# shivams15/navierstokessolver

Hardware: AMD Instinct MI355X
Metric: cell-updates/sec (MLUPS) + Poisson iters/sec, 4096^2 grid at 1/2/4/8 GPUs (higher is better)
Workload: dtype f64

## Files before the change

navierstokessolver_amd/csrc/ns_fps.hip:

```cpp
#include <hip/hip_ext.h>
#include <hip/hip_runtime.h>

#include <algorithm>

#include "ns_internal.h"

namespace nsg {

namespace {

struct cplx {
    double x, y;
};
__device__ inline cplx cadd(cplx a, cplx b) { return {a.x + b.x, a.y + b.y}; }
__device__ inline cplx csub(cplx a, cplx b) { return {a.x - b.x, a.y - b.y}; }
__device__ inline cplx cmul(cplx a, cplx b) { return {fma(a.x, b.x, -a.y * b.y), fma(a.x, b.y, a.y * b.x)}; }

__device__ inline double2 ld2(const double* p) { return *reinterpret_cast<const double2*>(p); }
__device__ inline void st2(double* p, double x, double y) { *reinterpret_cast<double2*>(p) = double2{x, y}; }

__device__ constexpr double C16[8] = {1.0, 0.92387953251128675613, 0.70710678118654752440, 0.38268343236508977173,
                                      0.0, -0.38268343236508977173, -0.70710678118654752440, -0.92387953251128675613};
__device__ constexpr double S16[8] = {0.0, 0.38268343236508977173, 0.70710678118654752440, 0.92387953251128675613,
                                      1.0, 0.92387953251128675613, 0.70710678118654752440, 0.38268343236508977173};
// ... 1351 lines not shown
        BR[w][0] = BR[w][1] = 1.0;
        if (c < a.nch) {
            double2 e = le[w];
            const double2 pp = lp[w];
            double2 bl = lb[w];
            if (a.m0e && k0 == 0) {
                const double sft = a.ny * *a.m0s;
                e.x -= sft * a.m0e[c];
                bl.x -= sft * a.m0b[c];
            }
            const double2 be = lbe[w], br = lbr[w];
            if (!a.mid_local) st2(a.ya + (size_t)c * a.ld + k0, Y[0], Y[1]);
            BX[w][0] = fma(be.x, Y[0], bl.x);
            BX[w][1] = fma(be.y, Y[1], bl.y);
            BR[w][0] = br.x;
            BR[w][1] = br.y;
            if (!a.mid_local) st2(a.cb + (size_t)c * a.ld + k0, BX[w][0], BX[w][1]);
            Y[0] = fma(pp.x, Y[0], e.x);
            Y[1] = fma(pp.y, Y[1], e.y);
        }
    }
    double GX[2] = {0.0, 0.0}, GR[2] = {1.0, 1.0};
#pragma unroll
    for (int w = FPS_G - 1; w >= 0; w--) {
        GX[0] = fma(BR[w][0], GX[0], BX[w][0]);
        GX[1] = fma(BR[w][1], GX[1], BX[w][1]);
        GR[0] = BR[w][0] * GR[0];
        GR[1] = BR[w][1] * GR[1];
    }
    st2(a.gb + (size_t)grp * a.ld + k0, GX[0], GX[1]);
    st2(a.gb + (size_t)(a.ngrp + grp) * a.ld + k0, GR[0], GR[1]);
}

template <bool GHOST>
__global__ void __launch_bounds__(64 * FPS_G) k_fps_t2b(FpsArgs a, double* __restrict__ f) {
    const int lane = threadIdx.x, w = __builtin_amdgcn_readfirstlane(threadIdx.y);
    const int k0 = 2 * (blockIdx.x * 64 + lane);
    const int grp = blockIdx.y, c = grp * FPS_G + w;
    const int li0 = c * FPS_M;
    const int rows = k0 < a.ny ? min(FPS_M, a.nxl - li0) : 0;
    ChunkRows cr;
    cr.load_wave(a, li0);
    if (rows <= 0) return;
    const double s0 = mode0_shift(a, k0);
    double2 yv[FPS_M];
#pragma unroll
    for (int t = 0; t < FPS_M; t++)
        yv[t] = ldf0(a, f, min(li0 + t, a.nxl - 1), k0, s0);
    const double2 yin = ld2(a.ya + (size_t)c * a.ld + k0);
    const double2 x0 = ld2(a.gx + (size_t)grp * a.ld + k0);
    double X[2] = {x0.x, x0.y};
    for (int q = FPS_G - 1; q > w; q--) {
        const int cq = grp * FPS_G + q;
        if (cq >= a.nch) continue;
        const double2 bx = ld2(a.cb + (size_t)cq * a.ld + k0), br = ld2(a.bt + (size_t)(a.nch + cq) * a.ld + k0);
        X[0] = fma(br.x, X[0], bx.x);
        X[1] = fma(br.y, X[1], bx.y);
    }
    if (GHOST && c == a.nch - 1 && a.i0 + a.nxl < a.nx) st2(f + (size_t)a.nxl * a.ld + k0, X[0], X[1]);
    const double mu[2] = {a.mu[k0], a.mu[k0 + 1]};
    const double2 r0 = ld2(a.rp0 + (size_t)c * a.ld + k0);
    double r[2] = {r0.x, r0.y}, y[2] = {yin.x, yin.y};
    double2 rv[FPS_M];
    const int pb = fps_prow_block(a);
    const bool fast = pb < a.nx;
    const double2 pinf = fast ? ld2(a.pinf + k0) : double2{0.0, 0.0};
// ... 529 lines not shown
    }
    if (a.cnt <= 0) return np;
    int n = -1;
    switch (lg) {
    case 4: n = div_pair<4>(k, a, st); break;
    case 5: n = div_pair<5>(k, a, st); break;
    case 6: n = div_pair<6>(k, a, st); break;
    case 7: n = div_pair<7>(k, a, st); break;
    case 8: n = div_pair<8>(k, a, st); break;
    case 9: n = div_pair<9>(k, a, st); break;
    case 10: n = div_pair<10>(k, a, st); break;
    case 11: n = div_pair<11>(k, a, st); break;
    case 12: n = div_pair<12>(k, a, st); break;
    case 13: n = div_pair<13>(k, a, st); break;
    default: return -1;
    }
    return n < 0 ? -1 : np;
}

bool fps_fuse_ok(const Knobs& k, int ny, int outE) { return ny == (1 << 14) ? fps_div_real(k, 14, outE) : fps_log2(ny) >= 0; }

void launch_fps_t1(const FpsArgs& a, const double* f, hipStream_t st) {
    hipLaunchKernelGGL(k_fps_t1, dim3((a.ny + 127) / 128, a.ngrp), dim3(64, FPS_G), 0, st, a, f);
}
void launch_fps_t2(const FpsArgs& a, double* f, hipStream_t st) {
    hipLaunchKernelGGL(k_fps_t2, dim3((a.ny + 127) / 128, a.ngrp), dim3(64, FPS_G), 0, st, a, f);
}
void launch_fps_t1b(const FpsArgs& a, const double* f, hipStream_t st) {
    hipLaunchKernelGGL(k_fps_t1b, dim3((a.ny + 127) / 128, a.ngrp), dim3(64, FPS_G), 0, st, a, f);
}
void launch_fps_mid(const FpsArgs& a, const double* f, hipStream_t st) {
    hipLaunchKernelGGL(k_fps_mid, dim3((a.ny + 127) / 128, a.ngrp), dim3(64), 0, st, a, f);
}
namespace {
__global__ void k_fps_oe_s0(const double* __restrict__ f, int row, int ld, int last, double* __restrict__ out) {
    if (threadIdx.x == 0) out[0] = last ? 2.0 * f[(size_t)row * ld] : 0.0;
}
}
void launch_fps_oe_s0(const double* f, int row, int ld, int last, double* out, hipStream_t st) {
    hipLaunchKernelGGL(k_fps_oe_s0, dim3(1), dim3(64), 0, st, f, row, ld, last, out);
}
void launch_fps_t2b(const FpsArgs& a, double* f, hipStream_t st) {
    if (a.ghost) hipLaunchKernelGGL(k_fps_t2b<true>, dim3((a.ny + 127) / 128, a.ngrp), dim3(64, FPS_G), 0, st, a, f);
    else hipLaunchKernelGGL(k_fps_t2b<false>, dim3((a.ny + 127) / 128, a.ngrp), dim3(64, FPS_G), 0, st, a, f);
}
void launch_fps_t3(const FpsArgs& a, double* f, hipStream_t st) {
    hipLaunchKernelGGL(k_fps_t3, dim3((a.ny + 127) / 128, a.ngrp), dim3(64, FPS_G), 0, st, a, f);
}
namespace {

__global__ __launch_bounds__(256) void k_cap_gemv(CapArgs a, const double* __restrict__ z) {
    extern __shared__ double gl[];
    const int M = a.m + a.border;
    for (int f = threadIdx.x; f < M; f += 256) gl[f] = f < a.m ? z[a.fi[f]] - z[a.fj[f]] : 0.0;
    __syncthreads();
    const int row = blockIdx.x * 4 + (threadIdx.x >> 6), lane = threadIdx.x & 63;
    if (row >= M) return;
    const double* cr = a.cinv + (size_t)row * M;
    double acc = 0.0;
    for (int k = lane; k < M; k += 64) acc = fma(cr[k], gl[k], acc);
    for (int off = 32; off > 0; off >>= 1) acc += __shfl_xor(acc, off, 64);
    if (lane == 0) a.y[row] = acc;
}

__global__ __launch_bounds__(256) void k_cap_scatter(CapArgs a, double* __restrict__ q, int mode) {
    const int c = blockIdx.x * 256 + threadIdx.x;
// ... 125 lines not shown
```

navierstokessolver_amd/csrc/ns_internal.h:

```cpp
#pragma once
#include <hip/hip_runtime.h>
#include <cstdint>
#include <vector>

#include "ns_knobs.h"

namespace nsg {

constexpr int HALO = 7;

constexpr int FC_IN = 1 << 20;
constexpr int FC_DEEP = 1 << 21;
constexpr int FC_BAND = 1 << 22;
constexpr int FC_INT = 31;
constexpr int MAX_EDGES = 31;
__host__ __device__ inline int fc_edge(int code, int k) { return (code >> (5 * k)) & 31; }
struct EdgeDev {
    int neu;
    int enx, eny;
    double c0, c1;
};

struct Geo {
    const int32_t* fc = nullptr;
    const EdgeDev* et = nullptr;
    int nx, ny;
    int i0, nxl;
    int ld;
    int neu[4];
    double c0[4], c1[4];
    int enx[4], eny[4];
    int sr0 = 0, sr1 = 1 << 30;
    int dsx = 0;
    const int* ecell = nullptr;
    int necell = 0;
};

struct Coef {
// ... 39 lines not shown
int launch_helm_sweep3(const Knobs& kn, const Geo& g, const Coef& c, double alpha, double omega, const double* u, const double* v,
                       double* uo, double* vo, const double* ru, const double* rv, hipStream_t st, int which,
                       double* part = nullptr);
int launch_helm_sweep2(const Knobs& kn, const Geo& g, const Coef& c, double alpha, double omega, const double* u, const double* v,
                       double* uo, double* vo, const double* ru, const double* rv, double* part, hipStream_t st,
                       int which = 3);

int launch_pois_rbsor_tiled(const Geo& g, const Coef& c, double omega, const double* phi, double* out,
                            const double* rp, const double* shift, double* part, hipStream_t st);
int launch_pois_jacobi_tiled(const Geo& g, const Coef& c, double omega, const double* in, double* out,
                             const double* rp, const double* shift, double* part, hipStream_t st);
void set_strip_rows(int L);
void set_compute_cus(int n);
int device_cus();
void lds_attr_once(const void* kern, int bytes);
void time_next_launch(hipEvent_t a, hipEvent_t b);
bool time_next_launch_pending();
bool take_launch_timing(hipEvent_t& a, hipEvent_t& b);
void set_strip_phase(int phase);
int launch_pois_residual(const Geo& g, const Coef& c, const double* phi, const double* rp,
                         const double* shift, double* part, hipStream_t st);
int launch_correct(const Knobs& kn, const Geo& g, const Coef& c, double dt, const double* us, const double* vs, double* u, double* v,
                   const double* phi, double* part, hipStream_t st);
bool correct_streams(const Knobs& kn, const Geo& g);
int launch_correct_guess(const Knobs& kn, const Geo& g, const Coef& c, double dt, const double* us, const double* vs, double* u,
                         double* v, const double* phi, double* part, const double* h1, const double* h2,
                         const double* h3, const double* gc, double* gout, hipStream_t st);
void launch_reduce_sum(const double* p, int n, int nv, double* out, hipStream_t st);
void launch_reduce_sum_segs(const double* p, int n, int nseg, double* out, hipStream_t st);
void launch_reduce_sum_min(const double* ps, int ns, int nvs, double* outs, const double* pm, int nm, int nvm,
                           double* outm, hipStream_t st);
void launch_reduce_min(const double* p, int n, int nv, double* out, hipStream_t st);
void launch_reduce_sum_mean(const double* p, int n, double* sums, double ncells, double* out, hipStream_t st);
void launch_finish_mean(const double* sums, double ncells, double* shift_and_bn2, hipStream_t st);
void launch_bus_reduce(const double* gathered, int P, int nv, int nsum, const int* dst, double* out, hipStream_t st);
int launch_sums(const Geo& g, const double* f, double* part, hipStream_t st);
void launch_axpby(const Geo& g, double a, const double* x, double b, const double* y, double* out, hipStream_t st,
                  double c = 0.0, const double* z = nullptr, double d = 0.0, const double* w = nullptr,
                  double e = 0.0, const double* v = nullptr);
int launch_area_sum(const Geo& g, const Coef& c, const double* b, double* part, hipStream_t st);
void launch_area_fix(const Geo& g, const Coef& c, double* b, const double* sab, const double* shift, double area,
                     double inv_area, double n, double* kshift, hipStream_t st);
void launch_fill_random(const Geo& g, double* phi, double* rp, uint64_t seed, hipStream_t st);


__host__ __device__ inline bool mg_can_coarsen(int nx, int ny) {
    return nx % 2 == 0 && ny % 2 == 0 && nx >= 4 && ny >= 4 && nx * ny > 16;
}

int launch_restrict(const Geo& gf, const Coef& cf, const double* phi, const double* b, const double* shift,
                    const Geo& gc, const Coef& cc, double* bc, double* pc, double* part, hipStream_t st);
void launch_prolong(const Geo& gf, double* phi, const Geo& gc, const double* ec, hipStream_t st);

int launch_pois_rbsor2_restrict(const Knobs& kn, const Geo& g, const Coef& c, double omega, const double* phi, double* out,
                                const double* rp, const double* shift, const Geo& gc, double* bc, double* pc,
                                double* part, hipStream_t st, bool zin = false);

int launch_pois_rbsor2_restrict_guess(const Knobs& kn, const Geo& g, const Coef& c, double omega, const double* phi, double* out,
                                      const double* rp, const double* shift, const Geo& gc, double* bc, double* pc,
                                      double* part, const double* h1, const double* h2, const double* h3,
                                      const double* gcoef, hipStream_t st);

int launch_pois_rbsor2_prolong(const Knobs& kn, const Geo& g, const Coef& c, double omega, const double* phi, double* out,
                               const double* rp, const double* shift, const Geo& gc, const double* ec,
                               double* part, hipStream_t st);

// ... 78 lines not shown
    double* s0 = nullptr;
    int s0_given = 0;
    const double *ptab = nullptr, *pinf = nullptr;
    int prow = 0, kfast = 1 << 30;
    const int* prowb = nullptr;
    int mid_local = 0;
    int ghost = 0;
};
struct FpsRank {
    const double* gath = nullptr;
    int P = 1, r = 0, stride = 0;
    const double *a1 = nullptr, *ge1 = nullptr;
    double ncells = 0.0;
    double* shift = nullptr;
    const double *bq = nullptr, *x1 = nullptr;
};
int fps_log2(int ny);
bool fps_idct_mask_ok(int ny);
bool fps_fuse_ok(const Knobs& kn, int ny, int outE);
int launch_fps_idct_masked(const Knobs& kn, const double* in, double* out, int nrows, int ny, int ld, const double* tw, const double* wk,
                           hipStream_t st, const int32_t* fcm);
int launch_fps_dct(const Knobs& kn, bool inverse, const double* in, const double* shift, double* out, int nrows, int ny, int ld,
                   const double* tw, const double* wk, hipStream_t st, int oe_pair = -1, const double* tw8 = nullptr);
int fps_log2x(int ny);
bool fps_gen_ok(int ny);
void launch_dense_mats(const double* C, const double* shy, double rsum, int N, double* F, double* G, hipStream_t st);
int launch_fps_div(const Knobs& kn, const Geo& g, const Coef& c, double dt, const double* u, const double* v, double* b, double* out,
                   double* part, int phase, const double* tw, const double* wk, hipStream_t st, int outE = 0);
void launch_fps_t1(const FpsArgs& a, const double* f, hipStream_t st);
void launch_fps_t2(const FpsArgs& a, double* f, hipStream_t st);
void launch_fps_t3(const FpsArgs& a, double* f, hipStream_t st);
void launch_fps_t1b(const FpsArgs& a, const double* f, hipStream_t st);
void launch_fps_mid(const FpsArgs& a, const double* f, hipStream_t st);
void launch_fps_t2b(const FpsArgs& a, double* f, hipStream_t st);
void launch_fps_oe_s0(const double* f, int row, int ld, int last, double* out, hipStream_t st);
void launch_fps_scan(const FpsArgs& a, bool backward, const FpsRank& R, double* rout, hipStream_t st);

struct CapArgs {
    int m = 0, ncell = 0, border = 0;
    const double* e1 = nullptr;
    const int *fi = nullptr, *fj = nullptr, *fk = nullptr, *fm = nullptr, *co = nullptr;
    const int4* cf = nullptr;
    const double* w = nullptr;
    double *cinv = nullptr, *y = nullptr;
};
constexpr size_t CAP_LDS_MAX = 8192;
hipError_t launch_cap_gemv(const CapArgs& a, const double* z, hipStream_t st);
void launch_cap_scatter(const CapArgs& a, double* q, int mode, hipStream_t st);
void launch_cap_axpy(const Geo& g, const CapArgs& a, double* x, const double* z, int set, hipStream_t st);
void launch_cap_fill(const Geo& g, double* q, double val, hipStream_t st);
void launch_cap_rhs(const Geo& g, const double* b, const double* shift, double* r, hipStream_t st);
void launch_cap_src(const CapArgs& a, double* q, int fprev, int f, hipStream_t st);
void launch_cap_col(const CapArgs& a, const double* z, int f, double* cmat, hipStream_t st);
void launch_gj_invert(double* A, int m, double* t, double* u, double* flag, int spd, hipStream_t st);

}
```

navierstokessolver_amd/csrc/ns_kernels.hip:

```cpp
#include "ns_internal.h"
#include <hip/hip_ext.h>

#include <cmath>
#include <cstdio>
#include <cstdlib>
#include <cstring>
#include <map>
#include <set>
#include <mutex>

#include <algorithm>

namespace nsg {

#ifndef LANE_DPP
#define LANE_DPP 1
#endif
__device__ __forceinline__ double lane_up1(double x) {
#if LANE_DPP
    const int lo = __double2loint(x), hi = __double2hiint(x);
    return __hiloint2double(__builtin_amdgcn_update_dpp(hi, hi, 0x138, 0xf, 0xf, false),
                            __builtin_amdgcn_update_dpp(lo, lo, 0x138, 0xf, 0xf, false));
#else
    return __shfl_up(x, 1, 64);
// ... 3804 lines not shown
    double m[4] = {INFINITY, INFINITY, INFINITY, INFINITY};
    for (int k = threadIdx.x; k < n; k += 1024)
#pragma unroll
        for (int v = 0; v < 4; v++)
            if (v < nv) m[v] = fmin(m[v], p[(size_t)k * nv + v]);
#pragma unroll
    for (int v = 0; v < 4; v++)
#pragma unroll
        for (int off = 32; off > 0; off >>= 1) m[v] = fmin(m[v], __shfl_xor(m[v], off, 64));
    const int wv = threadIdx.x >> 6, lane = threadIdx.x & 63;
    if (lane == 0)
#pragma unroll
        for (int v = 0; v < 4; v++) sh[wv][v] = m[v];
    __syncthreads();
    if (threadIdx.x < 4 && (int)threadIdx.x < nv) {
        double r = sh[0][threadIdx.x];
        for (int w = 1; w < 16; w++) r = fmin(r, sh[w][threadIdx.x]);
        out[threadIdx.x] = r;
    }
}
__global__ __launch_bounds__(1024) void k_reduce_min(const double* __restrict__ p, int n, int nv,
                                                     double* __restrict__ out) {
    __shared__ double sh[16][4];
    reduce_min_body(p, n, nv, out, sh);
}
__global__ __launch_bounds__(1024) void k_reduce_sum_min(const double* __restrict__ ps, int ns, int nvs,
                                                         double* __restrict__ outs, const double* __restrict__ pm,
                                                         int nm, int nvm, double* __restrict__ outm) {
    __shared__ double sh[1024];
    if (blockIdx.x == 0) reduce_sum_body(ps, ns, nvs, outs, sh);
    else reduce_min_body(pm, nm, nvm, outm, reinterpret_cast<double (*)[4]>(sh));
}

__global__ __launch_bounds__(1024) void k_reduce_sum_mean(const double* __restrict__ p, int n,
                                                          double* __restrict__ sums, double nc,
                                                          double* __restrict__ out) {
    __shared__ double sh[1024];
    double r[2];
    for (int v = 0; v < 2; v++) {
        double s = 0.0;
        for (int k = threadIdx.x; k < n; k += 1024) s += p[(size_t)k * 2 + v];
        r[v] = tree_sum_1024(s, sh);
        if (threadIdx.x == 0) sums[v] = r[v];
    }
    if (threadIdx.x == 0) {
        const double s = r[0], s2 = r[1];
        out[0] = s / nc;
        out[1] = fmax(s2 - s * s / nc, 0.0);
    }
}
__global__ void k_finish_mean(const double* __restrict__ sums, double n, double* __restrict__ out) {
    const double s = sums[0], s2 = sums[1];
    out[0] = s / n;
    out[1] = fmax(s2 - s * s / n, 0.0);
}

struct BusDst {
    int d[16];
};
__global__ void k_bus_reduce(const double* __restrict__ g, int P, int nv, int nsum, BusDst dst,
                             double* __restrict__ out) {
    const int t = threadIdx.x;
    if (t >= nv) return;
    double a = g[t];
    for (int q = 1; q < P; q++) {
        const double x = g[(size_t)q * nv + t];
// ... 1686 lines not shown
                                                     double* __restrict__ z, double* __restrict__ zg) {
    const int j = blockIdx.x * 256 + threadIdx.x;
    if (j >= ld) return;
    const double v = j < ny ? p[j] : 0.0;
    for (int r = blockIdx.y; r < rows; r += gridDim.y) z[(ptrdiff_t)r * ld + j] = v;
    if (zg && blockIdx.y == 0) zg[j] = v;
}

int launch_line_solve(const double* r, const Coef& c, int ny, double* p, hipStream_t st) {
    if (ny > LINE_CAP) return -1;
    lds_attr_once((const void*)k_line_solve, 4 * LINE_CAP * (int)sizeof(double));
    NS_LAUNCH(k_line_solve, dim3(1), dim3(1024), (size_t)4 * ny * sizeof(double), st, r, c.ps, c.pn, c.hy, ny, p);
    return 0;
}

void launch_line_extend(const double* p, const Geo& g, double* z, int rows, double* zg, hipStream_t st) {
    NS_LAUNCH(k_line_extend, dim3((g.ld + 255) / 256, std::min(rows, 256)), dim3(256), 0, st, p, g.ny, g.ld, rows, z,
              zg);
}

void launch_reduce_sum(const double* p, int n, int nv, double* out, hipStream_t st) {
    NS_LAUNCH(k_reduce_sum, dim3(1), dim3(1024), 0, st, p, n, nv, out);
}
void launch_reduce_sum_segs(const double* p, int n, int nseg, double* out, hipStream_t st) {
    NS_LAUNCH(k_reduce_sum_segs, dim3(1), dim3(1024), 0, st, p, n, nseg, out);
}
void launch_reduce_min(const double* p, int n, int nv, double* out, hipStream_t st) {
    NS_LAUNCH(k_reduce_min, dim3(1), dim3(1024), 0, st, p, n, nv, out);
}
void launch_reduce_sum_min(const double* ps, int ns, int nvs, double* outs, const double* pm, int nm, int nvm,
                           double* outm, hipStream_t st) {
    NS_LAUNCH(k_reduce_sum_min, dim3(2), dim3(1024), 0, st, ps, ns, nvs, outs, pm, nm, nvm, outm);
}
void launch_reduce_sum_mean(const double* p, int n, double* sums, double ncells, double* out, hipStream_t st) {
    NS_LAUNCH(k_reduce_sum_mean, dim3(1), dim3(1024), 0, st, p, n, sums, ncells, out);
}
void launch_bus_reduce(const double* gathered, int P, int nv, int nsum, const int* dst, double* out, hipStream_t st) {
    BusDst d{};
    for (int t = 0; t < nv && t < 16; t++) d.d[t] = dst[t];
    NS_LAUNCH(k_bus_reduce, dim3(1), dim3(64), 0, st, gathered, P, nv, nsum, d, out);
}
void launch_finish_mean(const double* sums, double ncells, double* out, hipStream_t st) {
    NS_LAUNCH(k_finish_mean, dim3(1), dim3(1), 0, st, sums, ncells, out);
}
int launch_sums(const Geo& g, const double* f, double* part, hipStream_t st) {
    const int rows = cell_rows(g);
    const dim3 cg = cell_grid(g, rows);
    NS_LAUNCH(k_sums, cg, dim3(64, 4), 0, st, g, f, part, rows);
    return (int)(cg.x * cg.y);
}
void launch_axpby(const Geo& g, double a, const double* x, double b, const double* y, double* out, hipStream_t st,
                  double c, const double* z, double d, const double* w, double e, const double* v) {
    NS_LAUNCH(k_axpby, cell_grid(g), dim3(64, 4), 0, st, g, a, x, b, y, c, z, d, w, e, v, out);
}
int launch_area_sum(const Geo& g, const Coef& c, const double* b, double* part, hipStream_t st) {
    const int rows = cell_rows(g);
    const dim3 cg = cell_grid(g, rows);
    NS_LAUNCH(k_area_sum, cg, dim3(64, 4), 0, st, g, c, b, part, rows);
    return (int)(cg.x * cg.y);
}
void launch_area_fix(const Geo& g, const Coef& c, double* b, const double* sab, const double* shift, double area,
                     double inv_area, double n, double* kshift, hipStream_t st) {
    NS_LAUNCH(k_area_fix, cell_grid(g), dim3(64, 4), 0, st, g, c, b, sab, shift, area, inv_area, n, kshift);
}
void launch_fill_random(const Geo& g, double* phi, double* rp, uint64_t seed, hipStream_t st) {
    NS_LAUNCH(k_fill_random, cell_grid(g), dim3(64, 4), 0, st, g, phi, rp, seed);
// ... 4 lines not shown
```

navierstokessolver_amd/csrc/ns_solver.cpp:

```cpp
#include <rccl/rccl.h>
#include <rocblas/rocblas.h>
#include <rocsolver/rocsolver.h>
#include <dlfcn.h>
#include <limits>

#include <algorithm>
#include <cmath>
#include <cstdarg>
#include <cstdio>
#include <cstring>
#include <map>
#include <string>
#include <vector>

#include "../../include/nsgpu.h"
#include "ns_internal.h"

namespace {

thread_local std::string g_err;

void set_err(const char* fmt, ...) {
    char buf[1024];
    va_list ap;
// ... 81 lines not shown
    int rank = 0, nranks = 1;
    ncclComm_t comm = nullptr;
    double ncells = 0;
    std::vector<hipEvent_t> ev;
    std::vector<char> evtag;
    std::vector<hipEvent_t> hev;
    int hn = 0;
    std::vector<int> hcomp;
    int helm_batch0 = 4, pois_batch0 = 8;
    int helm_next = 4;
    int helm_adapt = 1;
    int band_w = 128, band_sweeps = 6;
    int helm_probe = 0;
    int phi_extrap = 3;
    double mg_rate2 = 0.0;
    int mg_hist[4] = {-1, -1, -1, -1};
    double* phim = nullptr;
    double* phim2 = nullptr;
    double* phim3 = nullptr;
    double* phim4 = nullptr;
    double* phim_mem = nullptr;
    float* f32_mem = nullptr;
    float* f32[3] = {};
    int phim_valid = 0;
    int overlap = 1;
    int helm_b_pend = 0;
    struct Piggy { const nsg::Geo* g; double* f; int w; };
    Piggy piggy[4];
    int npiggy = 0;
    hipStream_t cst = nullptr;
    int comm_cus = 0, compute_cus = 0;
    hipEvent_t xev[2] = {nullptr, nullptr};
    hipEvent_t fev = nullptr;
    double* mm_host = nullptr;
    hipEvent_t mev = nullptr;
    int mm_pending = 0;
    int extrap_pending = 0;
    std::vector<MgLevel> lv;
    int mg_pre = 2, mg_post = 2, mg_coarse_iters = 0;
    double mg_omega_c = 1.0, mg_omega_s = 1.1;
    bool mg_coarse_lds = false;
    bool p_pending = false;
    bool gin_pending = false;
    const double* gin_src[4] = {nullptr, nullptr, nullptr, nullptr};
    double gin_c[4] = {0, 0, 0, 0};
    bool mg_direct = false;
    double* dmat = nullptr;
    const double *dP1 = nullptr, *dQ1 = nullptr, *dE = nullptr, *dP2 = nullptr, *dQ2 = nullptr;
    double* kv[9] = {};
    double* kv_mem = nullptr;
    double* lrow = nullptr;
    double* cvimg = nullptr;
    int cv_n = 0, cv_dn = 0;
    double* ksc = nullptr;
    bool pc_active = false;
    bool pc_timing = false;
    bool krylov_mg = false;
    int out_side = -1;
    bool consist = false;
    bool fps_xuni = true;
    bool fps_dense = false;
    rocblas_handle rb = nullptr;
    double *dense_mem = nullptr, *dF = nullptr, *dG = nullptr;
    double area = 0.0;
    double inv_area = 0.0;
    int32_t* fc_mem = nullptr;
// ... 675 lines not shown
            s->mask_helm_ok = 0;
        } else {
            s->mask_helm_next = sweeps;
            if (!first_ok) s->mask_helm_ok = 0;
        }
        return 0;
    }
    if (s->g.fc) {
        CHK(fetch(s));
        int iu = 0, iv = 0;
        const KrylovSolve ku{1, alpha, false, s->arr[NS_ARR_U], s->arr[NS_ARR_RU], nullptr, s->hs[S_HBN], "helmholtz u"};
        CHK(bicgstab(s, ku, &iu, resu));
        const KrylovSolve kw{1, alpha, false, s->arr[NS_ARR_V], s->arr[NS_ARR_RV], nullptr, s->hs[S_HBN + 1], "helmholtz v"};
        CHK(bicgstab(s, kw, &iv, resv));
        *its = std::max(iu, iv);
        return 0;
    }
    const double tol2 = s->rtol * s->rtol;
    if (s->k.helm_band && !s->k.tiled) CHK(helm_band(s, alpha));
    int sweeps = 0, batch = s->rp_h > 0 ? s->rp_h : s->helm_next, prev_at = -1;
    const int n0 = batch;
    double prev_r2 = -1;
    double first_r2 = -1, last_r2 = -1;
    int first_at = 0, last_at = 0;
    double* p0 = s->part + 2 * (size_t)nsg::max_partials(s->g) / 2;
    for (;;) {
        const int n = std::min(batch, s->max_iters - sweeps);
        const bool first = sweeps == 0 && n > 3 && (s->helm_probe == 0 || !s->helm_adapt);
        int nb0 = 0, at0 = 0, at = 0;
        const int nb = helm_sweeps(s, alpha, n, first ? p0 : nullptr, s->part, &nb0, &at0, &at);
        at += sweeps;
        sweeps += n;
        const bool ub = bus_on(s);
        nsg::launch_reduce_sum_segs(s->part, nb, 2, s->scal + (ub ? S_RESL : S_RES), s->st);
        if (first) nsg::launch_reduce_sum_segs(p0, nb0, 2, s->scal + (ub ? S_AUXL : S_AUX), s->st);
        static_assert(S_RES == S_HBN + 2, "the deferred RHS norms and the residuals in one all-reduce");
        if (ub) {
            CHK(bus(s));
        } else {
            if (s->hbn_pend) CHK(allreduce(s, s->scal + S_HBN, 4, ncclSum));
            else CHK(allreduce(s, s->scal + S_RES, 2, ncclSum));
            if (first) CHK(allreduce(s, s->scal + S_AUX, 2, ncclSum));
        }
        s->hbn_pend = false;
        CHK(fetch_begin(s));
        if (s->extrap_pending && !s->guess_ready && !(s->k.gin && gin_ok(s) && s->phim_valid > 0)) {
            s->extrap_pending = 0;
            CHK(extrapolate_phi(s));
        } else if (s->k.speculate && s->in_step) {
            CHK(divergence(s));
            s->k3_spec = 1;
        }
        CHK(fetch_end(s));
        const double r2u = s->hs[S_RES], r2v = s->hs[S_RES + 1];
        const double bu = s->hs[S_HBN], bv = s->hs[S_HBN + 1];
        const bool ok = s->rp_h > 0 || ((r2u <= tol2 * bu || r2u == 0.0) && (r2v <= tol2 * bv || r2v == 0.0));
        *resu = bu > 0 ? std::sqrt(r2u / bu) : std::sqrt(r2u);
        *resv = bv > 0 ? std::sqrt(r2v / bv) : std::sqrt(r2v);
        if (!std::isfinite(r2u) || !std::isfinite(r2v)) { set_err("Helmholtz residual is not finite"); *its = sweeps; return NS_EDIVERGE; }
        if (s->k.verbose) {
            if (first)
                fprintf(stderr, "nsgpu helmholtz: after %d sweeps rel. residual u %.3e v %.3e\n", at0,
                        std::sqrt(s->hs[S_AUX] / std::max(bu, 1e-300)), std::sqrt(s->hs[S_AUX + 1] / std::max(bv, 1e-300)));
            fprintf(stderr, "nsgpu helmholtz: after %d sweeps rel. residual u %.3e v %.3e\n", at, *resu, *resv);
        }
        const double r2 = std::max(r2u / std::max(bu, 1e-300), r2v / std::max(bv, 1e-300));
        if (first) {
// ... 986 lines not shown
        const double one = 1.0, zero = 0.0;
        if (dense_lib().dgemm(s->rb, rocblas_operation_none, rocblas_operation_none, g.ny, g.nxl, g.ny, &one, s->dF, g.ny,
                          s->arr[NS_ARR_RPHI], g.ld, &zero, F, g.ld) != rocblas_status_success) {
            set_err("direct Poisson solve: the dense forward transform (rocblas_dgemm) failed");
            return NS_EHIP;
        }
        if (t) HIPCHK(hipEventRecord(s->kev[3], s->st));
        fa.sh0 = fa1.sh0 = fam.sh0 = s->scal + S_SHIFT;
    } else if (!pre && nsg::launch_fps_dct(s->k, false, s->arr[NS_ARR_RPHI], oe ? nullptr : s->scal + S_SHIFT, F, g.nxl, g.ny,
                                           g.ld, s->fps_tw, s->fps_wk, s->st, oe_pair, s->fps_tw8) < 0) {
        set_err("direct Poisson solve: ny = %d is not a supported power of two", g.ny);
        return NS_EINVAL;
    }
    if (t) {
        if (!pre && !s->fps_dense) CHK(t_end(s, s->kev[2], s->kev[3]));
        HIPCHK(hipEventRecord(s->kev[4], s->st));
    }
    if (oe && s->nranks > 1) {
        nsg::launch_fps_oe_s0(F, g.nxl - 1, g.ld, g.i0 + g.nxl == g.nx ? 1 : 0, s->scal + S_OE, s->st);
        CHK(allreduce(s, s->scal + S_OE, 1, ncclSum));
        for (nsg::FpsArgs* q : {&fa, &fa1, &fam}) {
            q->s0 = s->scal + S_OE;
            q->s0_given = 1;
        }
    }
    if (s->fps_passes == 3) {
        nsg::launch_fps_t1(fa, F, s->st);
        CHK(fps_scan(s, false));
        nsg::launch_fps_t2(fa, F, s->st);
        CHK(fps_scan(s, true));
        nsg::launch_fps_t3(fa, F, s->st);
    } else {
        nsg::launch_fps_t1b(fa1, F, s->st);
        CHK(fps_scan(s, false));
        s->mean_pend = false;
        nsg::launch_fps_mid(fam, F, s->st);
        CHK(fps_scan(s, true));
        nsg::FpsArgs fa2 = fa;
        fa2.ghost = s->deep && s->in_step ? 1 : 0;
        nsg::launch_fps_t2b(fa2, F, s->st);
    }
    const int glo = s->fps_passes != 3 && s->deep && s->in_step && g.i0 > 0 ? 1 : 0;
    const int ghi = s->fps_passes != 3 && s->deep && s->in_step && g.i0 + g.nxl < g.nx ? 1 : 0;
    s->phi_ext = s->fps_passes != 3 && s->deep && s->in_step ? 1 : 0;
    if (t) {
        HIPCHK(hipEventRecord(s->kev[5], s->st));
        if (s->fps_dense) HIPCHK(hipEventRecord(s->kev[6], s->st));
        else CHK(t_begin(s, s->kev[6], s->kev[7]));
    }
    if (s->fps_dense) {
        const double one = 1.0, zero = 0.0;
        if (dense_lib().dgemm(s->rb, rocblas_operation_none, rocblas_operation_none, g.ny, g.nxl + glo + ghi, g.ny, &one,
                          s->dG, g.ny, F - (ptrdiff_t)glo * g.ld, g.ld, &zero,
                          s->arr[NS_ARR_PHI] - (ptrdiff_t)glo * g.ld, g.ld) != rocblas_status_success) {
            set_err("direct Poisson solve: the dense inverse transform (rocblas_dgemm) failed");
            return NS_EHIP;
        }
    } else {
        nsg::launch_fps_dct(s->k, true, F - (ptrdiff_t)glo * g.ld, nullptr, s->arr[NS_ARR_PHI] - (ptrdiff_t)glo * g.ld,
                            g.nxl + glo + ghi, g.ny, g.ld, s->fps_tw, s->fps_wk, s->st, -1, s->fps_tw8);
    }
    if (t) {
        if (s->fps_dense) HIPCHK(hipEventRecord(s->kev[7], s->st));
        else CHK(t_end(s, s->kev[6], s->kev[7]));
    }
    auto take_times = [&]() -> int {
        if (!t || !stt) return 0;
        HIPCHK(hipEventSynchronize(s->kev[7]));
        stt->t_fps_dct_ms += kev_ms(s, 2);
        stt->t_fps_tri_ms += kev_ms(s, 4);
// ... 850 lines not shown
    nsg::launch_reduce_sum(s->part, nb, 2, s->scal + S_AUX, s->st);
    nb = nsg::launch_sums(s->g, s->arr[NS_ARR_RV], s->part, s->st);
    nsg::launch_reduce_sum(s->part, nb, 2, s->scal + S_AUX + 2, s->st);
    CHK(allreduce(s, s->scal + S_AUX, 4, ncclSum));
    HIPCHK(hipMemcpyAsync(s->scal + S_HBN, s->scal + S_AUX + 1, sizeof(double), hipMemcpyDeviceToDevice, s->st));
    HIPCHK(hipMemcpyAsync(s->scal + S_HBN + 1, s->scal + S_AUX + 3, sizeof(double), hipMemcpyDeviceToDevice, s->st));
    return 0;
}

int rhs(ns_solver* s, bool defer_norm = false) {
    const bool t = s->timing && s->in_step;
    if (t) {
        CHK(ensure_kev(s));
        CHK(t_begin(s, s->kev[0], s->kev[1]));
    }
    int nb;
    if (s->deep && s->in_step) {
        const int e = s->deep_e, ld = s->g.ld;
        const HaloReq r[5] = {{&s->g, s->arr[NS_ARR_U], e + 2}, {&s->g, s->arr[NS_ARR_V], e + 2},
                              {&s->g, s->arr[NS_ARR_PHI], e + 1}, {&s->g, s->arr[NS_ARR_CU], e},
                              {&s->g, s->arr[NS_ARR_CV], e}};
        int lo = 0;
        const nsg::Geo gk = deep_geo(s, e, &lo);
        nb = overlapped(s, r, s->cu_ext >= e ? 3 : 5, [&]() {
            return nsg::launch_rhs(s->k, gk, s->c, s->dt, s->re, shp(s->arr[NS_ARR_U], lo, ld), shp(s->arr[NS_ARR_V], lo, ld),
                                   shp(s->arr[NS_ARR_PHI], lo, ld), shp(s->arr[NS_ARR_CU], lo, ld),
                                   shp(s->arr[NS_ARR_CV], lo, ld), shp(s->arr[NS_ARR_RU], lo, ld),
                                   shp(s->arr[NS_ARR_RV], lo, ld), s->part, s->st, e + 2);
        });
        s->cu_ext = e;
        s->u_ext = e + 2;
    } else if (s->corr_pend && s->in_step) {
        double* mm = s->part + 4 * (size_t)nsg::max_partials(s->g);
        nb = nsg::launch_rhs(s->k, s->g, s->c, s->dt, s->re, s->arr[NS_ARR_U], s->arr[NS_ARR_V], s->arr[NS_ARR_PHI],
                             s->arr[NS_ARR_CU], s->arr[NS_ARR_CV], s->arr[NS_ARR_RU], s->arr[NS_ARR_RV], s->part, s->st,
                             2, s->arr[NS_ARR_TMPU], s->arr[NS_ARR_TMPV], mm);
        if (nb < 0) { set_err("K1 with the deferred correction: launch refused"); return NS_EHIP; }
        std::swap(s->arr[NS_ARR_U], s->arr[NS_ARR_TMPU]);
        std::swap(s->arr[NS_ARR_V], s->arr[NS_ARR_TMPV]);
        s->corr_pend = 0;
        s->corr_k1 = 1;
        s->cu_ext = 0;
        if (nb < 0) return nb;
        if (t) CHK(t_end(s, s->kev[0], s->kev[1]));
        nsg::launch_reduce_sum_min(s->part, nb, 2, s->scal + S_HBN, mm, nb, 4, s->scal + S_MM, s->st);
        return 0;
    } else {
        const HaloReq r[3] = {{&s->g, s->arr[NS_ARR_U], 2}, {&s->g, s->arr[NS_ARR_V], 2}, {&s->g, s->arr[NS_ARR_PHI], 1}};
        nb = overlapped(s, r, 3, [&]() {
            return nsg::launch_rhs(s->k, s->g, s->c, s->dt, s->re, s->arr[NS_ARR_U], s->arr[NS_ARR_V], s->arr[NS_ARR_PHI],
                                   s->arr[NS_ARR_CU], s->arr[NS_ARR_CV], s->arr[NS_ARR_RU], s->arr[NS_ARR_RV], s->part,
                                   s->st);
        });
        s->cu_ext = 0;
    }
    if (nb < 0) return nb;
    if (t) CHK(t_end(s, s->kev[0], s->kev[1]));
    const bool ub = defer_norm && bus_on(s);
    nsg::launch_reduce_sum(s->part, nb, 2, s->scal + (ub ? S_HBNL : S_HBN), s->st);
    if (ub) {
    } else if (defer_norm && comm_on(s) && !s->g.fc) s->hbn_pend = true;
    else CHK(allreduce(s, s->scal + S_HBN, 2, ncclSum));
    return 0;
}

int correct_launch(ns_solver* s, double* part2) {
    const HaloReq r[1] = {{&s->g, s->arr[NS_ARR_PHI], 1}};
    const ExtrapPlan p = extrap_plan(s, s->cur_cycles);
    const bool guess = s->in_step && s->k.k5_guess && p.branch >= 1 && p.branch <= 3 && nsg::correct_streams(s->k, s->g);
    s->guess_ready = 0;
    const bool have = s->deep && s->phi_ext && s->in_step;
    const bool t5 = s->timing && s->in_step && !guess;
    if (t5) {
        CHK(ensure_kev(s));
        CHK(t_begin(s, s->kev[12], s->kev[13]));
    }
    const int nb = have ? [&]() {
        if (guess)
// ... 1448 lines not shown
```

Measured before the change: 15340.

## Fuse FPS forward scan, mid pass and backward scan into one kernel; defer K1 reductions

On a single rank, the forward group scan, the mid-chunk combine and the backward scan of the fast Poisson solver now run in one kernel, with per-mode group carries held in LDS, replacing three-plus separate launches. Separately, the K1 norm and min reductions are deferred and merged with the residual reduction into one four-block reduce kernel. Both changes aim to cut launch count and global round-trips in the Poisson tail. The costs are fewer blocks (ny/16) doing longer serial scans, and extra state that carries a pending reduction across phases.

```diff
diff --git a/navierstokessolver_amd/csrc/ns_fps.hip b/navierstokessolver_amd/csrc/ns_fps.hip
--- a/navierstokessolver_amd/csrc/ns_fps.hip
+++ b/navierstokessolver_amd/csrc/ns_fps.hip
@@ -1407,6 +1407,169 @@
     st2(a.gb + (size_t)(a.ngrp + grp) * a.ld + k0, GR[0], GR[1]);
 }
 
+constexpr int MS_MB = 16;
+constexpr int MS_NT = 512;
+template <int S, bool BACK, class LE, class LP, class SC>
+__device__ __forceinline__ void ms_scan(int ngrp, int ny, int kb, int tid, LE ldE, LP ldP, SC stC, double (*sE)[MS_MB],
+                                        double (*sP)[MS_MB], double (*sY)[MS_MB]) {
+    const int lane = tid % MS_MB, s = tid / MS_MB;
+    const int k = kb + lane;
+    constexpr int B = 8;
+    auto gq = [&](int q) { return BACK ? ngrp - 1 - q : q; };
+    if (S > 1 && ngrp >= 2 * S) {
+        const bool act = s < S && k < ny;
+        const int per = (ngrp + S - 1) / S, q0 = s * per, q1 = min(ngrp, q0 + per);
+        double AE = 0.0, AP = 1.0;
+        if (act) {
+            for (int qb = q0; qb < q1; qb += B) {
+                double E[B], P[B];
+#pragma unroll
+                for (int t = 0; t < B; t++) {
+                    const int q = qb + t, qc = min(q, q1 - 1);
+                    const double e = ldE(gq(qc), lane), pv = ldP(gq(qc), lane);
+                    E[t] = q < q1 ? e : 0.0;
+                    P[t] = q < q1 ? pv : 1.0;
+                }
+#pragma unroll
+                for (int t = 0; t < B; t++) {
+                    AE = fma(P[t], AE, E[t]);
+                    AP = P[t] * AP;
+                }
+            }
+        }
+        if (s < S) {
+            sE[s][lane] = AE;
+            sP[s][lane] = AP;
+        }
+        __syncthreads();
+        if (s == 0 && k < ny) {
+            double Y = 0.0;
+            for (int t = 0; t < S; t++) {
+                sY[t][lane] = Y;
+                Y = fma(sP[t][lane], Y, sE[t][lane]);
+            }
+        }
+        __syncthreads();
+        if (act) {
+            double Y = sY[s][lane];
+            for (int qb = q0; qb < q1; qb += B) {
+                double E[B], P[B];
+#pragma unroll
+                for (int t = 0; t < B; t++) {
+                    const int q = qb + t, qc = min(q, q1 - 1);
+                    const double e = ldE(gq(qc), lane), pv = ldP(gq(qc), lane);
+                    E[t] = q < q1 ? e : 0.0;
+                    P[t] = q < q1 ? pv : 1.0;
+                }
+#pragma unroll
+                for (int t = 0; t < B; t++) {
+                    const int q = qb + t;
+                    if (q < q1) {
+                        stC(gq(q), lane, Y);
+                        Y = fma(P[t], Y, E[t]);
+                    }
+                }
+            }
+        }
+    } else if (s == 0 && k < ny) {
+        double Y = 0.0;
+        for (int q0 = 0; q0 < ngrp; q0 += B) {
+            double E[B], P[B];
+#pragma unroll
+            for (int t = 0; t < B; t++) {
+                const int q = q0 + t, qc = min(q, ngrp - 1);
+                const double e = ldE(gq(qc), lane), pv = ldP(gq(qc), lane);
+                E[t] = q < ngrp ? e : 0.0;
+                P[t] = q < ngrp ? pv : 1.0;
+            }
+#pragma unroll
+            for (int t = 0; t < B; t++) {
+                const int q = q0 + t;
+                if (q < ngrp) {
+                    stC(gq(q), lane, Y);
+                    Y = fma(P[t], Y, E[t]);
+                }
+            }
+        }
+    }
+}
+template <int S>
+__global__ void __launch_bounds__(MS_NT) k_fps_midscan(FpsArgs a, const double* __restrict__ f) {
+    extern __shared__ double ms_lds[];
+    __shared__ double sE[S][MS_MB], sP[S][MS_MB], sY[S][MS_MB];
+    static_assert(MS_NT >= S * MS_MB, "k_fps_midscan: a thread per mode and segment");
+    const int tid = threadIdx.x, ngrp = a.ngrp, ld = a.ld, kb = blockIdx.x * MS_MB;
+    double* gc = ms_lds;
+    double* gbx = gc + (size_t)ngrp * MS_MB;
+    double* gbr = gbx + (size_t)ngrp * MS_MB;
+    ms_scan<S, false>(
+        ngrp, a.ny, kb, tid, [&](int grp, int lane) { return a.ga[(size_t)grp * ld + kb + lane]; },
+        [&](int grp, int lane) { return a.ga[(size_t)(ngrp + grp) * ld + kb + lane]; },
+        [&](int grp, int lane, double Y) { gc[grp * MS_MB + lane] = Y; }, sE, sP, sY);
+    __syncthreads();
+    constexpr int NP = MS_MB / 2;
+    for (int task = tid; task < NP * ngrp; task += MS_NT) {
+        const int pr = task % NP, grp = task / NP;
+        const int k0 = kb + 2 * pr;
+        if (k0 >= a.ny) continue;
+        if (a.outE && !a.s0_given && k0 == 0 && grp == 0) *a.s0 = mode0_shift(a, 0, f);
+        double Y[2] = {gc[grp * MS_MB + 2 * pr], gc[grp * MS_MB + 2 * pr + 1]};
+        double BX[FPS_G][2], BR[FPS_G][2];
+        double2 le[FPS_G], lp[FPS_G], lb[FPS_G], lbe[FPS_G], lbr[FPS_G];
+#pragma unroll
+        for (int w = 0; w < FPS_G; w++) {
+            const int c = min(grp * FPS_G + w, a.nch - 1);
+            le[w] = ld2(a.ca + (size_t)c * a.ld + k0);
+            lp[w] = ld2(a.ca + (size_t)(a.nch + c) * a.ld + k0);
+            lb[w] = ld2(a.cb + (size_t)c * a.ld + k0);
+            lbe[w] = ld2(a.bt + (size_t)c * a.ld + k0);
+            lbr[w] = ld2(a.bt + (size_t)(a.nch + c) * a.ld + k0);
+        }
+#pragma unroll
+        for (int w = 0; w < FPS_G; w++) {
+            const int c = grp * FPS_G + w;
+            BX[w][0] = BX[w][1] = 0.0;
+            BR[w][0] = BR[w][1] = 1.0;
+            if (c < a.nch) {
+                double2 e = le[w];
+                const double2 pp = lp[w];
+                double2 bl = lb[w];
+                if (a.m0e && k0 == 0) {
+                    const double sft = a.ny * *a.m0s;
+                    e.x -= sft * a.m0e[c];
+                    bl.x -= sft * a.m0b[c];
+                }
+                const double2 be = lbe[w], br = lbr[w];
+                st2(a.ya + (size_t)c * a.ld + k0, Y[0], Y[1]);
+                BX[w][0] = fma(be.x, Y[0], bl.x);
+                BX[w][1] = fma(be.y, Y[1], bl.y);
+                BR[w][0] = br.x;
+                BR[w][1] = br.y;
+                st2(a.cb + (size_t)c * a.ld + k0, BX[w][0], BX[w][1]);
+                Y[0] = fma(pp.x, Y[0], e.x);
+                Y[1] = fma(pp.y, Y[1], e.y);
+            }
+        }
+        double GX[2] = {0.0, 0.0}, GR[2] = {1.0, 1.0};
+#pragma unroll
+        for (int w = FPS_G - 1; w >= 0; w--) {
+            GX[0] = fma(BR[w][0], GX[0], BX[w][0]);
+            GX[1] = fma(BR[w][1], GX[1], BX[w][1]);
+            GR[0] = BR[w][0] * GR[0];
+            GR[1] = BR[w][1] * GR[1];
+        }
+        gbx[grp * MS_MB + 2 * pr] = GX[0];
+        gbx[grp * MS_MB + 2 * pr + 1] = GX[1];
+        gbr[grp * MS_MB + 2 * pr] = GR[0];
+        gbr[grp * MS_MB + 2 * pr + 1] = GR[1];
+    }
+    __syncthreads();
+    ms_scan<S, true>(
+        ngrp, a.ny, kb, tid, [&](int grp, int lane) { return gbx[grp * MS_MB + lane]; },
+        [&](int grp, int lane) { return gbr[grp * MS_MB + lane]; },
+        [&](int grp, int lane, double Y) { a.gx[(size_t)grp * ld + kb + lane] = Y; }, sE, sP, sY);
+}
+
 template <bool GHOST>
 __global__ void __launch_bounds__(64 * FPS_G) k_fps_t2b(FpsArgs a, double* __restrict__ f) {
     const int lane = threadIdx.x, w = __builtin_amdgcn_readfirstlane(threadIdx.y);
@@ -2002,6 +2165,12 @@
 void launch_fps_mid(const FpsArgs& a, const double* f, hipStream_t st) {
     hipLaunchKernelGGL(k_fps_mid, dim3((a.ny + 127) / 128, a.ngrp), dim3(64), 0, st, a, f);
 }
+bool launch_fps_midscan(const FpsArgs& a, const double* f, hipStream_t st) {
+    const size_t lds = 3 * (size_t)a.ngrp * MS_MB * sizeof(double);
+    if (!NS_TAILS || a.mid_local || lds > 48 * 1024 || a.ny % MS_MB != 0) return false;
+    hipLaunchKernelGGL(k_fps_midscan<FPS_SSEG>, dim3(a.ny / MS_MB), dim3(MS_NT), lds, st, a, f);
+    return true;
+}
 namespace {
 __global__ void k_fps_oe_s0(const double* __restrict__ f, int row, int ld, int last, double* __restrict__ out) {
     if (threadIdx.x == 0) out[0] = last ? 2.0 * f[(size_t)row * ld] : 0.0;
diff --git a/navierstokessolver_amd/csrc/ns_internal.h b/navierstokessolver_amd/csrc/ns_internal.h
--- a/navierstokessolver_amd/csrc/ns_internal.h
+++ b/navierstokessolver_amd/csrc/ns_internal.h
@@ -4,6 +4,10 @@
 #include <vector>
 
 #include "ns_knobs.h"
+
+#ifndef NS_TAILS
+#define NS_TAILS 1
+#endif
 
 namespace nsg {
 
@@ -109,6 +113,8 @@
                            double* outm, hipStream_t st);
 void launch_reduce_min(const double* p, int n, int nv, double* out, hipStream_t st);
 void launch_reduce_sum_mean(const double* p, int n, double* sums, double ncells, double* out, hipStream_t st);
+void launch_reduce_step(const double* pr, int nr, double* outr, const double* ps, int ns, double* outs, const double* pm,
+                        double* outm, hipStream_t st);
 void launch_finish_mean(const double* sums, double ncells, double* shift_and_bn2, hipStream_t st);
 void launch_bus_reduce(const double* gathered, int P, int nv, int nsum, const int* dst, double* out, hipStream_t st);
 int launch_sums(const Geo& g, const double* f, double* part, hipStream_t st);
@@ -253,6 +259,7 @@
 void launch_fps_t3(const FpsArgs& a, double* f, hipStream_t st);
 void launch_fps_t1b(const FpsArgs& a, const double* f, hipStream_t st);
 void launch_fps_mid(const FpsArgs& a, const double* f, hipStream_t st);
+bool launch_fps_midscan(const FpsArgs& a, const double* f, hipStream_t st);
 void launch_fps_t2b(const FpsArgs& a, double* f, hipStream_t st);
 void launch_fps_oe_s0(const double* f, int row, int ld, int last, double* out, hipStream_t st);
 void launch_fps_scan(const FpsArgs& a, bool backward, const FpsRank& R, double* rout, hipStream_t st);
diff --git a/navierstokessolver_amd/csrc/ns_kernels.hip b/navierstokessolver_amd/csrc/ns_kernels.hip
--- a/navierstokessolver_amd/csrc/ns_kernels.hip
+++ b/navierstokessolver_amd/csrc/ns_kernels.hip
@@ -3860,6 +3860,15 @@
     else reduce_min_body(pm, nm, nvm, outm, reinterpret_cast<double (*)[4]>(sh));
 }
 
+__global__ __launch_bounds__(1024) void k_reduce_step(const double* __restrict__ pr, int nr, double* __restrict__ outr,
+                                                      const double* __restrict__ ps, int ns, double* __restrict__ outs,
+                                                      const double* __restrict__ pm, double* __restrict__ outm) {
+    __shared__ double sh[1024];
+    if (blockIdx.x < 2) reduce_sum_body(pr + (size_t)blockIdx.x * nr, nr, 1, outr + blockIdx.x, sh);
+    else if (blockIdx.x == 2) reduce_sum_body(ps, ns, 2, outs, sh);
+    else reduce_min_body(pm, ns, 4, outm, reinterpret_cast<double (*)[4]>(sh));
+}
+
 __global__ __launch_bounds__(1024) void k_reduce_sum_mean(const double* __restrict__ p, int n,
                                                           double* __restrict__ sums, double nc,
                                                           double* __restrict__ out) {
@@ -5612,6 +5621,10 @@
                            double* outm, hipStream_t st) {
     NS_LAUNCH(k_reduce_sum_min, dim3(2), dim3(1024), 0, st, ps, ns, nvs, outs, pm, nm, nvm, outm);
 }
+void launch_reduce_step(const double* pr, int nr, double* outr, const double* ps, int ns, double* outs, const double* pm,
+                        double* outm, hipStream_t st) {
+    NS_LAUNCH(k_reduce_step, dim3(4), dim3(1024), 0, st, pr, nr, outr, ps, ns, outs, pm, outm);
+}
 void launch_reduce_sum_mean(const double* p, int n, double* sums, double ncells, double* out, hipStream_t st) {
     NS_LAUNCH(k_reduce_sum_mean, dim3(1), dim3(1024), 0, st, p, n, sums, ncells, out);
 }
diff --git a/navierstokessolver_amd/csrc/ns_solver.cpp b/navierstokessolver_amd/csrc/ns_solver.cpp
--- a/navierstokessolver_amd/csrc/ns_solver.cpp
+++ b/navierstokessolver_amd/csrc/ns_solver.cpp
@@ -137,6 +137,7 @@
     int comm_cus = 0, compute_cus = 0;
     hipEvent_t xev[2] = {nullptr, nullptr};
     hipEvent_t fev = nullptr;
+    int k1_red_nb = 0;
     double* mm_host = nullptr;
     hipEvent_t mev = nullptr;
     int mm_pending = 0;
@@ -878,7 +879,13 @@
         at += sweeps;
         sweeps += n;
         const bool ub = bus_on(s);
-        nsg::launch_reduce_sum_segs(s->part, nb, 2, s->scal + (ub ? S_RESL : S_RES), s->st);
+        if (s->k1_red_nb > 0 && !ub) {
+            nsg::launch_reduce_step(s->part, nb, s->scal + S_RES, s->part + 2 * (size_t)nsg::max_partials(s->g), s->k1_red_nb,
+                                    s->scal + S_HBN, s->part + 4 * (size_t)nsg::max_partials(s->g), s->scal + S_MM, s->st);
+            s->k1_red_nb = 0;
+        } else {
+            nsg::launch_reduce_sum_segs(s->part, nb, 2, s->scal + (ub ? S_RESL : S_RES), s->st);
+        }
         if (first) nsg::launch_reduce_sum_segs(p0, nb0, 2, s->scal + (ub ? S_AUXL : S_AUX), s->st);
         static_assert(S_RES == S_HBN + 2, "the deferred RHS norms and the residuals in one all-reduce");
         if (ub) {
@@ -1931,10 +1938,14 @@
         nsg::launch_fps_t3(fa, F, s->st);
     } else {
         nsg::launch_fps_t1b(fa1, F, s->st);
-        CHK(fps_scan(s, false));
-        s->mean_pend = false;
-        nsg::launch_fps_mid(fam, F, s->st);
-        CHK(fps_scan(s, true));
+        if (s->nranks == 1 && nsg::launch_fps_midscan(fam, F, s->st)) {
+            s->mean_pend = false;
+        } else {
+            CHK(fps_scan(s, false));
+            s->mean_pend = false;
+            nsg::launch_fps_mid(fam, F, s->st);
+            CHK(fps_scan(s, true));
+        }
         nsg::FpsArgs fa2 = fa;
         fa2.ghost = s->deep && s->in_step ? 1 : 0;
         nsg::launch_fps_t2b(fa2, F, s->st);
@@ -2851,8 +2862,9 @@
         s->u_ext = e + 2;
     } else if (s->corr_pend && s->in_step) {
         double* mm = s->part + 4 * (size_t)nsg::max_partials(s->g);
+        double* ps = NS_TAILS ? s->part + 2 * (size_t)nsg::max_partials(s->g) : s->part;
         nb = nsg::launch_rhs(s->k, s->g, s->c, s->dt, s->re, s->arr[NS_ARR_U], s->arr[NS_ARR_V], s->arr[NS_ARR_PHI],
-                             s->arr[NS_ARR_CU], s->arr[NS_ARR_CV], s->arr[NS_ARR_RU], s->arr[NS_ARR_RV], s->part, s->st,
+                             s->arr[NS_ARR_CU], s->arr[NS_ARR_CV], s->arr[NS_ARR_RU], s->arr[NS_ARR_RV], ps, s->st,
                              2, s->arr[NS_ARR_TMPU], s->arr[NS_ARR_TMPV], mm);
         if (nb < 0) { set_err("K1 with the deferred correction: launch refused"); return NS_EHIP; }
         std::swap(s->arr[NS_ARR_U], s->arr[NS_ARR_TMPU]);
@@ -2862,7 +2874,8 @@
         s->cu_ext = 0;
         if (nb < 0) return nb;
         if (t) CHK(t_end(s, s->kev[0], s->kev[1]));
-        nsg::launch_reduce_sum_min(s->part, nb, 2, s->scal + S_HBN, mm, nb, 4, s->scal + S_MM, s->st);
+        if (NS_TAILS) s->k1_red_nb = nb;
+        else nsg::launch_reduce_sum_min(ps, nb, 2, s->scal + S_HBN, mm, nb, 4, s->scal + S_MM, s->st);
         return 0;
     } else {
         const HaloReq r[3] = {{&s->g, s->arr[NS_ARR_U], 2}, {&s->g, s->arr[NS_ARR_V], 2}, {&s->g, s->arr[NS_ARR_PHI], 1}};
```

After: 15500, median of 6. 1.01x the previous value.
